# philips/janus

Hardware: AMD Instinct MI355X
Metric: reports prepared+aggregated/sec (helper, Prio3Histogram len=256) at 1/2/4/8 GPUs (higher is better)
Workload: dtype u32 limbs (Field128 mod-p integer arithmetic); 1 GPU; Prio3Histogram length=256 chunk_length=16 helper prepare_init+prepare_shares_to_prepare_message+prepare_next+aggregate, 1 segment; reports_per_gpu=1048576, global_batch=1048576, parallelism=dp1 (report shards; RCCL all-gather + mod-p combine)

## Files before the change

janus_amd/csrc/prio3_prepare.hip:

```cpp
#include <hip/hip_runtime.h>

#include <algorithm>

#include "prio3_host.h"
#include "prio3_query_sum.h"

#ifndef XOFD_BLOCK
#define XOFD_BLOCK 256
#endif
#ifndef XOFD_OCC
#define XOFD_OCC 3
#endif
template <class F>
__device__ __forceinline__ void xof_body(const DevParams& p, const InPtrs& in, const Scratch& sc,
                                         const uint32_t r) {
  if (r >= p.n) return;
  constexpr uint32_t ES = F::ES;
  uint32_t flag = p.force_slow;
  uint32_t nonce[4], km[4], kp[4], kb[4] = {0, 0, 0, 0};
  load16(in.nonces + 16 * (size_t)r, nonce);
  const uint8_t* hs = in.helper + (size_t)r * p.helper_share_len;
  load16(hs, km);
  load16(hs + 16, kp);
  const bool JR = p.jr_len > 0;
// ... 1051 lines not shown
  }
  return any != 0;
}

template <class F>
__device__ __forceinline__ void query_body(const DevParams& p, const InPtrs& in, const Scratch& sc,
                                           const OutPtrs& out, const uint32_t r) {
  typedef typename F::T T;
  if (r >= p.n) return;
  if (p.redo) {
    if (sc.flag[r] != 2) return;
  } else if (p.slow_defer && sc.flag[r]) {
    return;
  }
  const size_t ld = p.ld;
  const uint32_t A = p.arity;
  uint8_t status = PRIO3_STATUS_FINISHED;
  const T t = ldf<F>(sc.qr, 0, ld, r);
  T v, pt;
  if (!flp_query_lane<F>(p, sc.meas, sc.proofs, sc.jr, t, sc.Lbuf, sc.PVbuf, sc.acc, r, v, pt))
    status = PRIO3_STATUS_PREP_INIT;
  const uint8_t* lps = in.leader + (size_t)r * p.prep_share_len;
  bool decode_ok = true;
  auto lv = [&](uint32_t e) {
    T x = F::load(lps, e);
    if (!F::lt_p(x)) decode_ok = false;
    return x;
  };
  const T V0 = F::add(lv(0), v);
  T G = F::zero();
  if (p.kind == PRIO3_COUNT) {
    T a = F::add(lv(1), F::load(sc.acc, 0 * ld + r));
    T b = F::add(lv(2), F::load(sc.acc, 1 * ld + r));
    G = F::mul(a, b);
  } else if (p.kind == PRIO3_SUM) {
    T a = F::add(lv(1), F::load(sc.acc, r));
    G = F::sub(F::mul(a, a), a);
  } else {
    for (uint32_t j = 0; j < p.chunk; j++) {
      T a = F::add(lv(1 + 2 * j), F::load(sc.acc, (size_t)(2 * j) * ld + r));
      T b = F::add(lv(2 + 2 * j), F::load(sc.acc, (size_t)(2 * j + 1) * ld + r));
      G = F::add(G, F::mul(a, b));
    }
  }
  const T PT = F::add(lv(A + 1), pt);
  if (status == PRIO3_STATUS_FINISHED) {
    if (!decode_ok)
      status = PRIO3_STATUS_PREP_SHARE_DECODE;
    else if (!F::is_zero(V0) || !F::eq(G, PT))
      status = PRIO3_STATUS_PREP_MSG;
  }
  uint32_t msg[4] = {0, 0, 0, 0};
  if (p.jr_len > 0) {
    uint32_t lpart[4], hpart[4];
    load16(lps + (size_t)p.verifier_len * F::ES, lpart);
    uint4 hp = sc.part[r];
    hpart[0] = hp.x;
    hpart[1] = hp.y;
    hpart[2] = hp.z;
    hpart[3] = hp.w;
    KState s;
    kzero(s);
    Msg m;
    msg_zero(m);
    msg_dst(m, p.dst[6]);
    msg_bytes16(m, 25, lpart);
    msg_bytes16(m, 41, hpart);
    msg_absorb_final(s, m, 57);
    uint4 cor = sc.corrected[r];
    msg[0] = kword(s, 0);
    msg[1] = kword(s, 1);
    msg[2] = kword(s, 2);
    msg[3] = kword(s, 3);
    if (status == PRIO3_STATUS_FINISHED &&
        (msg[0] != cor.x || msg[1] != cor.y || msg[2] != cor.z || msg[3] != cor.w))
      status = PRIO3_STATUS_PREP_NEXT;
    if (status != PRIO3_STATUS_FINISHED) msg[0] = msg[1] = msg[2] = msg[3] = 0;
    ((uint4*)out.prep_msgs)[r] = make_uint4(msg[0], msg[1], msg[2], msg[3]);
  }
  out.status[r] = status;
  if (p.kind == PRIO3_SUM) {
    T acc = F::zero(), pw = F::one();
    for (uint32_t i = 0; i < p.meas_len; i++) {
      acc = F::add(acc, F::mul(pw, ldf<F>(sc.meas, i, ld, r)));
      pw = F::add(pw, pw);
    }
    F::store(sc.out, r, acc);
  } else if (p.kind == PRIO3_SUMVEC) {
    for (uint32_t e = 0; e < p.out_len; e++) {
      T acc = F::zero(), pw = F::one();
      for (uint32_t b = 0; b < p.bits; b++) {
        acc = F::add(acc, F::mul(pw, ldf<F>(sc.meas, e * p.bits + b, ld, r)));
        pw = F::add(pw, pw);
      }
      F::store(sc.out, (size_t)e * ld + r, acc);
    }
  }
}
template <class F>
__global__ __launch_bounds__(256) void k_query(DevParams p, InPtrs in, Scratch sc, OutPtrs out) {
  query_body<F>(p, in, sc, out, blockIdx.x * blockDim.x + threadIdx.x);
}

template <class F>
__global__ __launch_bounds__(256) void k_prep_gen(DevParams p, InPtrs in, Scratch sc, OutPtrs out) {
  const uint32_t r = blockIdx.x * blockDim.x + threadIdx.x;
  xof_body<F>(p, in, sc, r);
  query_body<F>(p, in, sc, out, r);
}

template <class F>
__global__ __launch_bounds__(64) void k_slow_redo_gen(DevParams p, InPtrs in, Scratch sc,
                                                      OutPtrs out) {
  const uint32_t r0 = (blockIdx.x * blockDim.x + threadIdx.x) * REDO_RPL;
  if (r0 >= p.n || !redo_any(p, sc, r0)) return;
  const uint8_t* fl = sc.flag + r0;
  for (uint32_t i = 0; i < REDO_RPL && r0 + i < p.n; i++)
    if (fl[i]) {
      xof_slow_one<F>(p, in, sc, r0 + i);
      query_body<F>(p, in, sc, out, r0 + i);
    }
}

template <int GS>
__global__ __launch_bounds__(256) void k_query_ps(DevParams p, InPtrs in, Scratch sc,
                                                  OutPtrs out) {
  typedef Fp128 F;
  typedef f128 T;
  const uint32_t r = blockIdx.x * blockDim.x + threadIdx.x;
  if (r >= p.n) return;
  const size_t ld = p.ld;
  const uint32_t P = p.P, A = p.arity, C = p.chunk, M = p.meas_len, K = p.calls;
  uint8_t status = PRIO3_STATUS_FINISHED;
  const T t = ldf<F>(sc.qr, 0, ld, r);
  {
    T tp = t;
    for (uint32_t l = 0; l < p.logP; l++) tp = F::mul(tp, tp);
    if (F::eq(tp, F::one())) status = PRIO3_STATUS_PREP_INIT;
  }
  {
    T pw = FC<F>::invP(p);
    for (uint32_t e = 0; e < P; e++) {
      F::store(sc.Lbuf, (size_t)bitrev(e, p.logP) * ld + r, pw);
      pw = F::mul(pw, t);
    }
    dft_lane<F>(p, sc.Lbuf, r, P, p.logP);
    for (uint32_t e = 0; e < P; e++) {
      T q = ldf<F>(sc.proofs, A + e, ld, r);
      if (e + P < p.glen) q = F::add(q, ldf<F>(sc.proofs, A + e + P, ld, r));
      F::store(sc.PVbuf, (size_t)bitrev(e, p.logP) * ld + r, q);
    }
    dft_lane<F>(p, sc.PVbuf, r, P, p.logP);
  }
  auto Lc = [&](uint32_t c) { return ldf<F>(sc.Lbuf, (P - c) & (P - 1), ld, r); };
  T pt = F::zero();
  for (uint32_t e = p.glen; e-- > 0;) pt = F::add(F::mul(pt, t), ldf<F>(sc.proofs, A + e, ld, r));
  const T r0 = ldf<F>(sc.jr, 0, ld, r);
  T rC = F::one();
  for (uint32_t j = 0; j < C; j++) rC = F::mul(rC, r0);
  T sumL = F::zero(), range = F::zero();
  {
    T rk = F::one();
    for (uint32_t k = 0; k < K; k++) {
      const T L = Lc(k + 1);
      sumL = F::add(sumL, L);
      range = F::add(range, ldf<F>(sc.PVbuf, k + 1, ld, r));
      F::store(sc.beta, (size_t)k * ld + r, F::mul(L, rk));
      rk = F::mul(rk, rC);
    }
  }
  const T L0 = Lc(0);
  const T half = FC<F>::half(p);
  const T halfL = F::mul(half, sumL);
  const uint8_t* lps = in.leader + (size_t)r * p.prep_share_len;
  bool decode_ok = true;
  auto lv = [&](uint32_t e) {
    T x = F::load(lps, e);
    if (!F::lt_p(x)) decode_ok = false;
    return x;
  };
  T S = F::zero(), G = F::zero(), rj = r0;
  const T Z = F::zero();
  for (uint32_t jg = 0; jg < C; jg += GS) {
    T Aa[GS], Bb[GS];
#pragma unroll
    for (int q = 0; q < GS; q++) Aa[q] = Bb[q] = Z;
    auto ldm = [&](uint32_t k, int q) {
      const uint32_t i = k * C + jg + (uint32_t)q;
      return ldf<F>(sc.meas, (jg + q < C && i < M) ? i : 0, ld, r);
    };
    T be_n = ldf<F>(sc.beta, 0, ld, r), L_n = Lc(1), mn[GS];
#pragma unroll
    for (int q = 0; q < GS; q++) mn[q] = ldm(0, q);
#pragma unroll 1
    for (uint32_t k = 0; k < K; k++) {
      const T be = be_n, L = L_n;
      T mc[GS];
#pragma unroll
      for (int q = 0; q < GS; q++) mc[q] = mn[q];
      const uint32_t kn = k + 1 < K ? k + 1 : k;
      be_n = ldf<F>(sc.beta, kn, ld, r);
      L_n = Lc(kn + 1);
#pragma unroll
      for (int q = 0; q < GS; q++) mn[q] = ldm(kn, q);
      const uint32_t base = k * C + jg;
#pragma unroll
      for (int q = 0; q < GS; q++) {
        const bool valid = (jg + q < C) && (base + q < M);
        const T m = F::sel(valid, mc[q], Z);
        Aa[q] = F::add(Aa[q], F::mul(be, m));
        Bb[q] = F::add(Bb[q], F::mul(L, m));
        S = F::add(S, m);
      }
    }
#pragma unroll
    for (int q = 0; q < GS; q++) {
      const uint32_t j = jg + q;
      const bool valid = j < C;
      const uint32_t jj = valid ? j : 0;
      const T f0 = F::add(F::mul(ldf<F>(sc.proofs, 2 * jj, ld, r), L0), F::mul(rj, Aa[q]));
      const T f1 = F::sub(F::add(F::mul(ldf<F>(sc.proofs, 2 * jj + 1, ld, r), L0), Bb[q]), halfL);
      const T prod = F::mul(F::add(lv(1 + 2 * jj), f0), F::add(lv(2 + 2 * jj), f1));
      G = F::add(G, F::sel(valid, prod, Z));
      rj = F::sel(valid, F::mul(rj, r0), rj);
    }
  }
  T v;
  if (p.kind == PRIO3_SUMVEC) {
    v = range;
  } else {
    const T r1 = ldf<F>(sc.jr, 1, ld, r);
    v = F::add(F::mul(r1, range), F::mul(F::mul(r1, r1), F::sub(S, half)));
  }
  const T V0 = F::add(lv(0), v);
  const T PT = F::add(lv(A + 1), pt);
  if (status == PRIO3_STATUS_FINISHED) {
    if (!decode_ok)
      status = PRIO3_STATUS_PREP_SHARE_DECODE;
    else if (!F::is_zero(V0) || !F::eq(G, PT))
      status = PRIO3_STATUS_PREP_MSG;
  }
  uint32_t lpart[4], hpart[4];
  load16(lps + (size_t)p.verifier_len * F::ES, lpart);
  {
    uint4 hp = sc.part[r];
    hpart[0] = hp.x;
    hpart[1] = hp.y;
    hpart[2] = hp.z;
    hpart[3] = hp.w;
  }
  KState s;
  kzero(s);
  Msg mm;
  msg_zero(mm);
  msg_dst(mm, p.dst[6]);
  msg_bytes16(mm, 25, lpart);
  msg_bytes16(mm, 41, hpart);
  msg_absorb_final(s, mm, 57);
  uint4 cor = sc.corrected[r];
  uint32_t msg[4] = {kword(s, 0), kword(s, 1), kword(s, 2), kword(s, 3)};
  if (status == PRIO3_STATUS_FINISHED &&
      (msg[0] != cor.x || msg[1] != cor.y || msg[2] != cor.z || msg[3] != cor.w))
    status = PRIO3_STATUS_PREP_NEXT;
  if (status != PRIO3_STATUS_FINISHED) msg[0] = msg[1] = msg[2] = msg[3] = 0;
  ((uint4*)out.prep_msgs)[r] = make_uint4(msg[0], msg[1], msg[2], msg[3]);
  out.status[r] = status;
  if (p.kind == PRIO3_SUMVEC) {
    for (uint32_t e = 0; e < p.out_len; e++) {
      T acc = F::zero(), pw = F::one();
      for (uint32_t b = 0; b < p.bits; b++) {
        acc = F::add(acc, F::mul(pw, ldf<F>(sc.meas, e * p.bits + b, ld, r)));
        pw = F::add(pw, pw);
      }
      F::store(sc.out, (size_t)e * ld + r, acc);
    }
  }
}

template <int GS, int PP, int LEADER = 0>
__device__ __forceinline__ void query_h_body(const DevParams& p, const InPtrs& in, const Scratch& sc,
                                             const OutPtrs& out, const uint32_t r) {
  typedef Fp128 F;
  typedef f128 T;
  constexpr int LOGP = PP <= 2 ? 1 : PP <= 4 ? 2 : PP <= 8 ? 3 : PP <= 16 ? 4 : 5;
  if (r >= p.n) return;
  if constexpr (!LEADER) {
    if (p.redo) {
      if (sc.flag[r] != 2) return;
    } else if (p.slow_defer && sc.flag[r]) {
      return;
    }
  } else {
    if (p.redo) {
      if (!sc.flag[r]) return;
    } else if (p.slow_defer && sc.flag[r]) {
      return;
    }
  }
  const size_t ld = p.ld;
  const uint32_t A = p.arity, C = p.chunk, M = p.meas_len, K = p.calls;
  uint8_t status = LEADER ? out.status[r] : PRIO3_STATUS_FINISHED;
  uint8_t* lout = LEADER ? out.prep_msgs + (size_t)r * p.prep_share_len : nullptr;
  const T t = ldf<F>(sc.qr, 0, ld, r);
  T L0, sumL = F::zero();
  auto store_L = [&](int idx, const T& val) {
    const uint32_t c = (uint32_t)((PP - idx) & (PP - 1));
    if (c == 0) {
      L0 = val;
    } else if (c <= K) {
      F::store(sc.Lbuf, (size_t)c * ld + r, val);
      sumL = F::add(sumL, val);
    }
  };
  if constexpr (PP <= 16) {
    T x[PP];
    T pw = FC<F>::invP(p);
#pragma unroll
    for (int e = 0; e < PP; e++) {
      x[__builtin_bitreverse32(e) >> (32 - LOGP)] = pw;
      pw = F::mul(pw, t);
    }
    if (F::eq(pw, FC<F>::invP(p))) status = PRIO3_STATUS_PREP_INIT;
    dft_reg<PP, LOGP>(p, x, 1);
#pragma unroll
    for (int k = 0; k < PP; k++) store_L(k, x[k]);
  } else {
    static_assert(PP == 32, "PP must be <= 32");
    T t8 = t;
#pragma unroll
    for (int i = 0; i < 3; i++) t8 = F::mul(t8, t8);
    const T t16 = F::mul(t8, t8);
    const T t32 = F::mul(t16, t16);
    if (F::eq(t32, F::one())) status = PRIO3_STATUS_PREP_INIT;
    const T ip = FC<F>::invP(p);
    const T a = F::add(F::one(), t16), b = F::sub(F::one(), t16);
    const T c = F::mul(t8, a), wd = F::mul(F::mul(t8, b), F::from_words(p.tw128[8]));
#pragma unroll
    for (int ph = 0; ph < 4; ph++) {
      const T g = ph == 0 ? F::add(a, c) : ph == 1 ? F::add(b, wd) : ph == 2 ? F::sub(a, c)
                                                                              : F::sub(b, wd);
      T x[8];
      T pw = F::mul(ip, g);
      const T ratio = ph == 0 ? t : F::mul(t, F::from_words(p.tw128[ph]));
#pragma unroll
      for (int e = 0; e < 8; e++) {
        x[__builtin_bitreverse32(e) >> 29] = pw;
        if (e + 1 < 8) pw = F::mul(pw, ratio);
      }
      dft_reg<8, 3>(p, x, 4);
#pragma unroll
      for (int k = 0; k < 8; k++) store_L(4 * k + ph, x[k]);
    }
  }
  T pt = F::zero(), range;
  {
    constexpr int GLEN = 2 * (PP - 1) + 1, NB = (GLEN + 7) / 8;
    T pw[8];
    pw[0] = F::one();
    pw[1] = t;
#pragma unroll
    for (int i = 2; i < 8; i++) pw[i] = F::mul(pw[i - 1], t);
    const T t8b = F::mul(pw[7], t);
    mac128 R;
    mac_zero(R);
    auto ldc = [&](int e) { return ldf<F>(sc.proofs, A + (e < GLEN ? e : 0), ld, r); };
    T cb[8];
#pragma unroll
    for (int i = 0; i < 8; i++) cb[i] = ldc(8 * (NB - 1) + i);
#pragma unroll 1
    for (int q = NB - 1; q >= 0; q--) {
      T cn[8];
      const int qn = q > 0 ? q - 1 : 0;
#pragma unroll
      for (int i = 0; i < 8; i++) cn[i] = ldc(8 * qn + i);
      mac128 S;
      mac_zero(S);
#pragma unroll
      for (int i = 0; i < 8; i++) {
        const int e = 8 * q + i;
        if (e < GLEN) {
          mac_add(S, cb[i], pw[i]);
          mac_add(R, cb[i], F::from_words(p.sigma128[e & (PP - 1)]));
        }
        cb[i] = cn[i];
      }
      const T sq = mac_reduce_f(S);
      pt = q == NB - 1 ? sq : F::add(F::mul(pt, t8b), sq);
    }
    range = mac_reduce_f(R);
  }
  const T r0 = ldf<F>(sc.jr, 0, ld, r);
  {
    T rC = F::one(), sq = r0;
    for (uint32_t e = C; e; e >>= 1) {
      if (e & 1) rC = F::mul(rC, sq);
      if (e > 1) sq = F::mul(sq, sq);
    }
    T rk = F::one();
    for (uint32_t k0 = 0; k0 < K; k0 += 8) {
      T lb[8];
#pragma unroll
      for (int q = 0; q < 8; q++) lb[q] = ldf<F>(sc.Lbuf, k0 + q < K ? k0 + q + 1 : 1, ld, r);
#pragma unroll
      for (int q = 0; q < 8; q++) {
        if (k0 + q < K) {
          F::store(sc.beta, (size_t)(k0 + q) * ld + r, F::mul(lb[q], rk));
          rk = F::mul(rk, rC);
        }
      }
    }
  }
  const T half = FC<F>::half(p);
  const T halfL = F::mul(half, sumL);
  const uint8_t* lps = in.leader + (size_t)r * p.prep_share_len;
  bool decode_ok = true;
  auto lv = [&](uint32_t e) {
    T x = F::load(lps, e);
    if (!F::lt_p(x)) decode_ok = false;
    return x;
  };
  sum128 Ssum;
  sum_zero(Ssum);
  T G = F::zero(), rj = r0;
  for (uint32_t jg = 0; jg < C; jg += GS) {
    mac128 Aa[GS], Bb[GS];
    T mc[GS];
#pragma unroll
    for (int q = 0; q < GS; q++) {
      mac_zero(Aa[q]);
      mac_zero(Bb[q]);
    }
    auto fetch = [&](uint32_t k, T* dst) {
#pragma unroll
      for (int q = 0; q < GS; q++) {
        const uint32_t i = k * C + jg + q;
        const bool valid = (k < K) && (jg + q < C) && (i < M);
        const uint32_t msk = valid ? 0xffffffffu : 0u;
        const uint4 v = ((const uint4*)sc.meas)[(size_t)(valid ? i : 0) * ld + r];
        dst[q] = mk128(v.x & msk, v.y & msk, v.z & msk, v.w & msk);
      }
    };
    fetch(0, mc);
    T be = ldf<F>(sc.beta, 0, ld, r), Lk = ldf<F>(sc.Lbuf, 1, ld, r);
#pragma unroll 1
    for (uint32_t k = 0; k < K; k++) {
      T mn[GS];
      fetch(k + 1, mn);
      const uint32_t kn = k + 1 < K ? k + 1 : k;
      const T be_n = ldf<F>(sc.beta, kn, ld, r), L_n = ldf<F>(sc.Lbuf, kn + 1, ld, r);
#pragma unroll
      for (int q = 0; q < GS; q++) {
        mac_add(Aa[q], be, mc[q]);
        mac_add(Bb[q], Lk, mc[q]);
        sum_add(Ssum, mc[q]);
      }
#pragma unroll
      for (int q = 0; q < GS; q++) mc[q] = mn[q];
      be = be_n;
      Lk = L_n;
    }
    mac128 Gq;
    mac_zero(Gq);
#pragma unroll
    for (int q = 0; q < GS; q++) {
      const uint32_t j = jg + q;
      if (j < C) {
        mac_add(Bb[q], ldf<F>(sc.proofs, 2 * j + 1, ld, r), L0);
        const T f1 = F::sub(mac_reduce_f(Bb[q]), halfL);
        const T Aq = mac_reduce_f(Aa[q]);
        mac128 F0;
        mac_zero(F0);
        mac_add(F0, ldf<F>(sc.proofs, 2 * j, ld, r), L0);
        mac_add(F0, rj, Aq);
        const T f0 = mac_reduce_f(F0);
        if constexpr (LEADER) {
          F::store(lout, 1 + 2 * j, f0);
          F::store(lout, 2 + 2 * j, f1);
        } else {
          mac_add(Gq, F::add(lv(1 + 2 * j), f0), F::add(lv(2 + 2 * j), f1));
        }
        rj = F::mul(rj, r0);
      }
    }
    if constexpr (!LEADER) G = F::add(G, mac_reduce_f(Gq));
  }
  const T S = sum_reduce(Ssum);
  T v;
  if (p.kind == PRIO3_SUMVEC) {
    v = range;
  } else {
    const T r1 = ldf<F>(sc.jr, 1, ld, r);
    v = F::add(F::mul(r1, range), F::mul(F::mul(r1, r1), F::sub(S, half)));
  }
  if constexpr (LEADER) {
    F::store(lout, 0, v);
    F::store(lout, A + 1, pt);
    *(uint4*)(lout + (size_t)p.verifier_len * F::ES) = sc.part[r];
    out.status[r] = status;
  } else {
  const T V0 = F::add(lv(0), v);
  const T PT = F::add(lv(A + 1), pt);
  if (status == PRIO3_STATUS_FINISHED) {
    if (!decode_ok)
      status = PRIO3_STATUS_PREP_SHARE_DECODE;
    else if (!F::is_zero(V0) || !F::eq(G, PT))
      status = PRIO3_STATUS_PREP_MSG;
  }
  uint32_t lpart[4], msg[4];
  load16(lps + (size_t)p.verifier_len * F::ES, lpart);
  if (!prep_msg_check(p, in, sc, r, lpart, msg) && status == PRIO3_STATUS_FINISHED)
    status = PRIO3_STATUS_PREP_NEXT;
  if (status != PRIO3_STATUS_FINISHED) msg[0] = msg[1] = msg[2] = msg[3] = 0;
  ((uint4*)out.prep_msgs)[r] = make_uint4(msg[0], msg[1], msg[2], msg[3]);
  out.status[r] = status;
  }
  if (p.kind == PRIO3_SUMVEC) {
    for (uint32_t e = 0; e < p.out_len; e++) {
      T acc = F::zero(), pw = F::one();
      for (uint32_t b = 0; b < p.bits; b++) {
        acc = F::add(acc, F::mul(pw, ldf<F>(sc.meas, e * p.bits + b, ld, r)));
        pw = F::add(pw, pw);
      }
      F::store(sc.out, (size_t)e * ld + r, acc);
    }
  }
}
template <int GS, int PP, int LEADER = 0>
__global__ __launch_bounds__(256, 3) void k_query_h(DevParams p, InPtrs in, Scratch sc,
                                                  OutPtrs out) {
  query_h_body<GS, PP, LEADER>(p, in, sc, out, blockIdx.x * blockDim.x + threadIdx.x);
}

template <bool FUSE, bool PULL = false>
__global__ __launch_bounds__(XOFD_BLOCK, 3) void k_prep_h(DevParams p, InPtrs in, Scratch sc,
                                                   OutPtrs out) {
  const uint32_t r = blockIdx.x * blockDim.x + threadIdx.x;
  xofd_body<FUSE, false, PULL>(p, in, sc, r);
  query_h_body<2, 32>(p, in, sc, out, r);
}

template <int PP>
__global__ __launch_bounds__(256, 3) void k_leader_prep(DevParams p, InPtrs in, Scratch sc,
                                                        OutPtrs out, uint32_t* wpart,
                                                        uint32_t* wseg) {
  const uint32_t r = blockIdx.x * blockDim.x + threadIdx.x;
  leader_jr_body(p, in, sc, out.status, wpart, wseg, r);
  query_h_body<2, PP, 1>(p, in, sc, out, r);
}

template <int NPH>
__global__ __launch_bounds__(256, 3) void k_prep_sum(DevParams p, InPtrs in, Scratch sc,
                                                     OutPtrs out) {
  const uint32_t r = blockIdx.x * blockDim.x + threadIdx.x;
  xofd_body<false, false>(p, in, sc, r);
  qsum::query_sum_body<NPH, 0>(p, in, sc, out, r);
}

template <int PP>
__global__ __launch_bounds__(64) void k_slow_redo(DevParams p, InPtrs in, Scratch sc, OutPtrs out) {
  const uint32_t r0 = (blockIdx.x * blockDim.x + threadIdx.x) * REDO_RPL;
  if (r0 >= p.n || !redo_any(p, sc, r0)) return;
  const uint8_t* fl = sc.flag + r0;
  for (uint32_t i = 0; i < REDO_RPL && r0 + i < p.n; i++)
    if (fl[i]) {
      xof_slow_one<Fp128>(p, in, sc, r0 + i);
      query_h_body<2, PP>(p, in, sc, out, r0 + i);
    }
}

template <int NPH>
__global__ __launch_bounds__(64) void k_slow_redo_sum(DevParams p, InPtrs in, Scratch sc,
                                                      OutPtrs out) {
  const uint32_t r0 = (blockIdx.x * blockDim.x + threadIdx.x) * REDO_RPL;
  if (r0 >= p.n || !redo_any(p, sc, r0)) return;
  const uint8_t* fl = sc.flag + r0;
  for (uint32_t i = 0; i < REDO_RPL && r0 + i < p.n; i++)
    if (fl[i]) {
      xof_slow_one<Fp128>(p, in, sc, r0 + i);
      qsum::query_sum_body<NPH, 0>(p, in, sc, out, r0 + i);
    }
}


static void fp_sub_sizes(const prio3_engine* e, uint32_t n, uint32_t cap, bool wide,
                         uint32_t& nsub, uint32_t& sub) {
  nsub = (n + cap - 1) / cap;
  sub = std::min(cap, (((n + nsub - 1) / nsub) + 255) & ~255u);
  if (wide && e->fp_round && nsub > 1) {
    const uint32_t Q = (uint32_t)e->n_cu * 4u * 2u * 8u;
    const uint32_t s2 = sub / Q * Q;
    if (s2 > 0 && n - (nsub - 1) * s2 <= cap) sub = s2;
  }
}

template <class F>
static void launch_xof_slow(const prio3_engine* e, const DevParams& p, const InPtrs& in,
                            const Scratch& sc, hipStream_t st) {
  (void)e;
  k_xof_slow<F><<<slow_blocks(p.n), 64, 0, st>>>(p, in, sc);
}

bool fusable(const prio3_engine* e) {
  return e->fuse_acc && e->dp.kind == PRIO3_HISTOGRAM && e->dp.jr_len &&
         (42 + e->dp.meas_len * 16) / 168 >= 2;
}

static int ensure_side_streams(prio3_engine* e) {
  while (e->side.size() < 2) {
    hipStream_t s2;
    hipEvent_t j;
    HIPCHK(hipStreamCreateWithFlags(&s2, hipStreamNonBlocking));
    HIPCHK(hipEventCreateWithFlags(&j, hipEventDisableTiming));
    e->side.push_back(s2);
    e->side_ev.push_back(j);
  }
  if (!e->fork_ev) HIPCHK(hipEventCreateWithFlags(&e->fork_ev, hipEventDisableTiming));
  return PRIO3_OK;
}

static bool prep_fused_takes(const prio3_engine* e, const DevParams& dp, bool fuse) {
  if (e->force_generic) return false;
  const bool ps = dp.kind == PRIO3_HISTOGRAM || dp.kind == PRIO3_SUMVEC;
  const bool dual = dp.es == 16 && dp.jr_len && (42 + dp.meas_len * 16) / 168 >= 2;
  if (dp.kind == PRIO3_SUM) return dual && !fuse && query_sum_takes(dp);
  return ps && dual && dp.P == 32;
}

enum : int { DEFER_NONE = 0, DEFER_QH = 1, DEFER_SUM = 2, DEFER_GEN64 = 3 };
static int launch_prepare(prio3_engine* e, const DevParams& base, uint32_t c0, uint32_t n,
                          InPtrs in, OutPtrs out, Scratch sc, hipStream_t st, bool fuse,
                          int* deferred, bool pair = false) {
  DevParams dp = base;
  dp.n = n;
  dp.force_slow = (uint32_t)e->force_slow;
  dp.slow_defer = 0;
  dp.redo = 0;
  const size_t es = dp.es;
  in.nonces += 16 * (size_t)c0;
  if (in.pub) in.pub += (size_t)dp.public_share_len * c0;
  in.helper += (size_t)dp.helper_share_len * c0;
  in.leader += (size_t)dp.prep_share_len * c0;
  if (in.vk_slot) in.vk_slot += c0;
  out.prep_msgs += (size_t)(dp.kind == PRIO3_SUMVEC_F64_MP ? 32 : 16) * c0;
  out.status += c0;
  void** soa[] = {&sc.meas, &sc.proofs, &sc.jr, &sc.qr, &sc.Lbuf, &sc.PVbuf, &sc.acc, &sc.out,
                  &sc.beta};
  for (auto q : soa)
    if (*q) *q = (uint8_t*)*q + es * c0;
  sc.part += c0;
  sc.corrected += c0;
  sc.flag += c0;
  if (sc.seg) sc.seg += c0;
  if (sc.wseg) sc.wseg += c0 / 64;
  if (sc.wpart) sc.wpart += (size_t)(c0 / 64) * dp.meas_len * 8;
  const uint32_t blocks = (n + 255) / 256;
  const uint32_t xblocks = (n + XOFD_BLOCK - 1) / XOFD_BLOCK;
  if (dp.kind == PRIO3_SUMVEC_F64_MP) {
    int rc = PRIO3_OK;
    TIMED(e, st, "k_mp64_prepare", (rc = launch_mp64(e, n, dp.ld, in, out, sc, st)));
    return rc;
  }
  if (dp.kind == PRIO3_FPVEC_BOUNDED_L2) {
    uint32_t nsub, sub;
    const bool qwide = !e->force_generic && fpvec_query_wide_takes(dp);
    fp_sub_sizes(e, n, dp.ld, qwide, nsub, sub);
    for (uint32_t si = 0; si < nsub; si++) {
      const uint32_t s0 = si * sub;
      DevParams q = dp;
      q.n = si + 1 < nsub ? sub : n - s0;
      InPtrs qi = in;
      qi.nonces += 16 * (size_t)s0;
      qi.pub += (size_t)dp.public_share_len * s0;
      qi.helper += (size_t)dp.helper_share_len * s0;
      qi.leader += (size_t)dp.prep_share_len * s0;
      if (qi.vk_slot) qi.vk_slot += s0;
      OutPtrs qo = out;
      qo.prep_msgs += 16 * (size_t)s0;
      qo.status += s0;
      Scratch qs = sc;
      qs.out = (uint8_t*)sc.out + es * s0;
      const uint32_t qb = (q.n + 255) / 256;
      const bool dual = (42 + dp.meas_len * 16) / 168 >= 2;
      q.trunc_xof = dual ? 1u : 0u;
      bool paired = false;
      if (dual) TIMED(e, st, "k_xof_pair", (paired = launch_xof_pair(q, qi, qs, st)));
      if (!paired && dual)
        TIMED(e, st, "k_xofd",
              (k_xofd<false, true><<<(q.n + XOFD_BLOCK - 1) / XOFD_BLOCK, XOFD_BLOCK, 0, st>>>(
                  q, qi, qs)));
      else if (!paired)
        TIMED(e, st, "k_xof", (k_xof<Fp128><<<qb, 256, 0, st>>>(q, qi, qs)));
      TIMED(e, st, "k_xof_slow", launch_xof_slow<Fp128>(e, q, qi, qs, st));
      if (qwide)
        TIMED(e, st, "k_query_fpw", launch_fpvec_query(q, qi, qs, qo, st, true, false));
      else
        TIMED(e, st, "k_query_fp", launch_fpvec_query(q, qi, qs, qo, st, false, false));
    }
    return PRIO3_OK;
  }
  if (dp.es == 16) {
    const bool ps = dp.kind == PRIO3_HISTOGRAM || dp.kind == PRIO3_SUMVEC;
    const bool wide = ps && !e->force_generic && dp.P != 32 && query_wide_takes(dp);
    const bool dual = dp.jr_len && (42 + dp.meas_len * 16) / 168 >= 2;
    dp.trunc_xof = dp.kind == PRIO3_SUMVEC && wide && dual && !fuse ? 1u : 0u;
    if (prep_fused_takes(e, dp, fuse)) {
      dp.slow_defer = 1u;
      if (dp.kind == PRIO3_SUM) {
        if (deferred) *deferred = DEFER_SUM;
        switch (dp.P) {
          case 16: TIMED(e, st, "k_prep_sum", (k_prep_sum<1><<<blocks, 256, 0, st>>>(dp, in, sc, out))); break;
          case 32: TIMED(e, st, "k_prep_sum", (k_prep_sum<2><<<blocks, 256, 0, st>>>(dp, in, sc, out))); break;
          case 64: TIMED(e, st, "k_prep_sum", (k_prep_sum<4><<<blocks, 256, 0, st>>>(dp, in, sc, out))); break;
          default: TIMED(e, st, "k_prep_sum", (k_prep_sum<8><<<blocks, 256, 0, st>>>(dp, in, sc, out))); break;
        }
      } else {
        if (deferred) *deferred = DEFER_QH;
        const bool pl = in.leader_src != nullptr;
        bool paired = false;
        if (pair)
          TIMED(e, st, "k_prep_hp", (paired = launch_prep_pair(dp, in, sc, out, st, fuse, pl)));
        if (paired) {
        } else if (fuse && pl)
          TIMED(e, st, "k_prep_h", (k_prep_h<true, true><<<xblocks, XOFD_BLOCK, 0, st>>>(dp, in, sc, out)));
        else if (fuse)
          TIMED(e, st, "k_prep_h", (k_prep_h<true><<<xblocks, XOFD_BLOCK, 0, st>>>(dp, in, sc, out)));
        else if (pl)
          TIMED(e, st, "k_prep_h", (k_prep_h<false, true><<<xblocks, XOFD_BLOCK, 0, st>>>(dp, in, sc, out)));
        else
          TIMED(e, st, "k_prep_h", (k_prep_h<false><<<xblocks, XOFD_BLOCK, 0, st>>>(dp, in, sc, out)));
      }
      return PRIO3_OK;
    }
    if (dual) {
      if (fuse)
        TIMED(e, st, "k_xofd", (k_xofd<true><<<xblocks, XOFD_BLOCK, 0, st>>>(dp, in, sc)));
      else if (dp.trunc_xof)
        TIMED(e, st, "k_xofd", (k_xofd<false, true><<<xblocks, XOFD_BLOCK, 0, st>>>(dp, in, sc)));
      else
        TIMED(e, st, "k_xofd", (k_xofd<false><<<xblocks, XOFD_BLOCK, 0, st>>>(dp, in, sc)));
    } else {
      TIMED(e, st, "k_xof_a", (k_xof_a<Fp128><<<blocks, 256, 0, st>>>(dp, in, sc)));
      TIMED(e, st, "k_jrpart", (k_jrpart<false><<<blocks, 256, 0, st>>>(dp, in, sc)));
    }
    const bool qh_path =
        ps && !e->force_generic && !wide && (dp.P == 32 || dp.P == 16 || dp.P == 8);
    dp.slow_defer = qh_path ? 1u : 0u;
    if (qh_path && deferred) *deferred = DEFER_QH;
    if (!qh_path) TIMED(e, st, "k_xof_slow", launch_xof_slow<Fp128>(e, dp, in, sc, st));
    bool done = false;
    if (wide) TIMED(e, st, "k_query_w", (done = launch_query_wide(dp, in, sc, out, st)));
    if (done) {
    } else if (qh_path && dp.P == 32)
      TIMED(e, st, "k_query_h", (k_query_h<2, 32><<<blocks, 256, 0, st>>>(dp, in, sc, out)));
    else if (qh_path && dp.P == 16)
      TIMED(e, st, "k_query_h", (k_query_h<2, 16><<<blocks, 256, 0, st>>>(dp, in, sc, out)));
    else if (qh_path && dp.P == 8)
      TIMED(e, st, "k_query_h", (k_query_h<2, 8><<<blocks, 256, 0, st>>>(dp, in, sc, out)));
    else if (ps)
      TIMED(e, st, "k_query_ps", (k_query_ps<4><<<blocks, 256, 0, st>>>(dp, in, sc, out)));
    else {
      bool qs = false;
      if (!e->force_generic && query_sum_takes(dp))
        TIMED(e, st, "k_query_sum", (qs = launch_query_sum(dp, in, sc, out, st)));
      if (!qs) TIMED(e, st, "k_query", (k_query<Fp128><<<blocks, 256, 0, st>>>(dp, in, sc, out)));
    }
  } else {
    dp.slow_defer = 1u;
    if (deferred) *deferred = DEFER_GEN64;
    TIMED(e, st, "k_prep_gen", (k_prep_gen<Fp64><<<blocks, 256, 0, st>>>(dp, in, sc, out)));
  }
  return PRIO3_OK;
}

static int launch_slow_redo(prio3_engine* e, const DevParams& base, uint32_t n, InPtrs in,
                            OutPtrs out, Scratch sc, hipStream_t st, int family) {
  DevParams dp = base;
  dp.n = n;
  dp.force_slow = (uint32_t)e->force_slow;
  dp.trunc_xof = 0;
  dp.slow_defer = 1;
  dp.redo = 1;
  const uint32_t g = redo_blocks(n);
  if (family == DEFER_GEN64) {
    TIMED(e, st, "k_slow_redo", (k_slow_redo_gen<Fp64><<<g, 64, 0, st>>>(dp, in, sc, out)));
  } else if (family == DEFER_SUM) {
    switch (dp.P) {
      case 16: TIMED(e, st, "k_slow_redo", (k_slow_redo_sum<1><<<g, 64, 0, st>>>(dp, in, sc, out))); break;
      case 32: TIMED(e, st, "k_slow_redo", (k_slow_redo_sum<2><<<g, 64, 0, st>>>(dp, in, sc, out))); break;
      case 64: TIMED(e, st, "k_slow_redo", (k_slow_redo_sum<4><<<g, 64, 0, st>>>(dp, in, sc, out))); break;
// ... 196 lines not shown
```

Before: 177.9 million reports/s.

## Spill live values to scratch and pipeline measurement loads with scalar offsets

Values that stay live across the long inner loop (L0, halfL, pt, range) now go to scratch buffers and are reloaded afterward, which lowers register pressure. Row loads use a per-lane base address plus a wave-uniform offset taken with readfirstlane, so address arithmetic can live in scalar registers. The inner loop is rewritten as a software pipeline with a remainder prologue and an unrolled steady state. The finalization loads for proofs, leader shares and jr are issued early so their latency is hidden. The cost is extra global memory traffic and reliance on compiler barriers and offsets being wave-uniform.

```diff
diff --git a/janus_amd/csrc/prio3_prepare.hip b/janus_amd/csrc/prio3_prepare.hip
--- a/janus_amd/csrc/prio3_prepare.hip
+++ b/janus_amd/csrc/prio3_prepare.hip
@@ -1377,11 +1377,11 @@
   uint8_t status = LEADER ? out.status[r] : PRIO3_STATUS_FINISHED;
   uint8_t* lout = LEADER ? out.prep_msgs + (size_t)r * p.prep_share_len : nullptr;
   const T t = ldf<F>(sc.qr, 0, ld, r);
-  T L0, sumL = F::zero();
+  T sumL = F::zero();
   auto store_L = [&](int idx, const T& val) {
     const uint32_t c = (uint32_t)((PP - idx) & (PP - 1));
     if (c == 0) {
-      L0 = val;
+      F::store(sc.Lbuf, r, val);
     } else if (c <= K) {
       F::store(sc.Lbuf, (size_t)c * ld + r, val);
       sumL = F::add(sumL, val);
@@ -1464,6 +1464,8 @@
     }
     range = mac_reduce_f(R);
   }
+  F::store(sc.PVbuf, (size_t)1 * ld + r, pt);
+  F::store(sc.PVbuf, (size_t)2 * ld + r, range);
   const T r0 = ldf<F>(sc.jr, 0, ld, r);
   {
     T rC = F::one(), sq = r0;
@@ -1486,7 +1488,7 @@
     }
   }
   const T half = FC<F>::half(p);
-  const T halfL = F::mul(half, sumL);
+  F::store(sc.PVbuf, r, F::mul(half, sumL));
   const uint8_t* lps = in.leader + (size_t)r * p.prep_share_len;
   bool decode_ok = true;
   auto lv = [&](uint32_t e) {
@@ -1497,69 +1499,133 @@
   sum128 Ssum;
   sum_zero(Ssum);
   T G = F::zero(), rj = r0;
+  uint64_t lane = (uint64_t)sc.meas + (uint64_t)r * F::ES;
+  asm("" : "+v"(lane));
   for (uint32_t jg = 0; jg < C; jg += GS) {
     mac128 Aa[GS], Bb[GS];
-    T mc[GS];
 #pragma unroll
     for (int q = 0; q < GS; q++) {
       mac_zero(Aa[q]);
       mac_zero(Bb[q]);
     }
-    auto fetch = [&](uint32_t k, T* dst) {
+    constexpr int WIRE_AHEAD = 1;
+    struct wire_ops {
+      T m[GS];
+      T be, L;
+    };
+    auto ldrow = [&](const void* base, uint32_t e) {
+      const uint64_t off = ((uint64_t)base - (uint64_t)sc.meas) + (uint64_t)e * ld * F::ES;
+      const uint64_t offu =
+          ((uint64_t)(uint32_t)__builtin_amdgcn_readfirstlane((int)(uint32_t)(off >> 32)) << 32) |
+          (uint32_t)__builtin_amdgcn_readfirstlane((int)(uint32_t)off);
+      typedef uint32_t u32x4 __attribute__((ext_vector_type(4)));
+      const u32x4 v = *(const __attribute__((address_space(1))) u32x4*)(lane + offu);
+      return mk128(v.x, v.y, v.z, v.w);
+    };
+    const uint32_t Klast = K ? K - 1 : 0;
+    auto issue = [&](uint32_t k, wire_ops& s) {
 #pragma unroll
       for (int q = 0; q < GS; q++) {
         const uint32_t i = k * C + jg + q;
         const bool valid = (k < K) && (jg + q < C) && (i < M);
+        s.m[q] = ldrow(sc.meas, i & (valid ? 0xffffffffu : 0u));
+      }
+      const uint32_t kc = min(k, Klast);
+      s.be = ldrow(sc.beta, kc);
+      s.L = ldrow(sc.Lbuf, kc + 1);
+    };
+    auto use = [&](uint32_t k, wire_ops& s) {
+#pragma unroll
+      for (int q = 0; q < GS; q++)
+        asm volatile(""
+                     : "+v"(s.m[q].w[0]), "+v"(s.m[q].w[1]), "+v"(s.m[q].w[2]), "+v"(s.m[q].w[3])
+                     :
+                     : "memory");
+#pragma unroll
+      for (int q = 0; q < GS; q++) {
+        const bool valid = (jg + q < C) && (k * C + jg + q < M);
         const uint32_t msk = valid ? 0xffffffffu : 0u;
-        const uint4 v = ((const uint4*)sc.meas)[(size_t)(valid ? i : 0) * ld + r];
-        dst[q] = mk128(v.x & msk, v.y & msk, v.z & msk, v.w & msk);
+        const T mc = mk128(s.m[q].w[0] & msk, s.m[q].w[1] & msk, s.m[q].w[2] & msk,
+                           s.m[q].w[3] & msk);
+        mac_add(Aa[q], s.be, mc);
+        mac_add(Bb[q], s.L, mc);
+        sum_add(Ssum, mc);
       }
     };
-    fetch(0, mc);
-    T be = ldf<F>(sc.beta, 0, ld, r), Lk = ldf<F>(sc.Lbuf, 1, ld, r);
+    constexpr int NS = WIRE_AHEAD + 1;
+    wire_ops ws[NS];
+    uint32_t k = __builtin_amdgcn_readfirstlane(0);
+    asm volatile("" : "+s"(k));
+#pragma unroll
+    for (int u = 0; u < WIRE_AHEAD; u++) issue(k + u, ws[u]);
 #pragma unroll 1
-    for (uint32_t k = 0; k < K; k++) {
-      T mn[GS];
-      fetch(k + 1, mn);
-      const uint32_t kn = k + 1 < K ? k + 1 : k;
-      const T be_n = ldf<F>(sc.beta, kn, ld, r), L_n = ldf<F>(sc.Lbuf, kn + 1, ld, r);
-#pragma unroll
-      for (int q = 0; q < GS; q++) {
-        mac_add(Aa[q], be, mc[q]);
-        mac_add(Bb[q], Lk, mc[q]);
-        sum_add(Ssum, mc[q]);
-      }
-#pragma unroll
-      for (int q = 0; q < GS; q++) mc[q] = mn[q];
-      be = be_n;
-      Lk = L_n;
-    }
+    for (uint32_t e = K % NS; e; e--, k++) {
+      issue(k + WIRE_AHEAD, ws[WIRE_AHEAD]);
+      use(k, ws[0]);
+#pragma unroll
+      for (int u = 0; u < WIRE_AHEAD; u++) ws[u] = ws[u + 1];
+    }
+#pragma unroll 1
+    for (; k < K; k += NS) {
+#pragma unroll
+      for (int u = 0; u < NS; u++) {
+        issue(k + u + WIRE_AHEAD, ws[(u + WIRE_AHEAD) % NS]);
+        use(k + u, ws[u]);
+      }
+    }
+    T sd[2 * GS], lw[2 * GS], r0f;
+    auto fin_load = [&](int q) {
+      const uint32_t jc = jg + q < C ? jg + q : jg;
+      if constexpr (!LEADER) {
+        lw[2 * q] = F::load(lps, 1 + 2 * jc);
+        lw[2 * q + 1] = F::load(lps, 2 + 2 * jc);
+      }
+    };
+    const T L0 = ldrow(sc.Lbuf, 0), halfL = ldrow(sc.PVbuf, 0);
+#pragma unroll
+    for (int q = 0; q < GS; q++) {
+      const uint32_t jc = jg + q < C ? jg + q : jg;
+      sd[2 * q + 1] = ldrow(sc.proofs, 2 * jc + 1);
+      sd[2 * q] = ldrow(sc.proofs, 2 * jc);
+    }
+    fin_load(0);
+    asm volatile("" ::: "memory");
     mac128 Gq;
     mac_zero(Gq);
 #pragma unroll
     for (int q = 0; q < GS; q++) {
       const uint32_t j = jg + q;
-      if (j < C) {
-        mac_add(Bb[q], ldf<F>(sc.proofs, 2 * j + 1, ld, r), L0);
-        const T f1 = F::sub(mac_reduce_f(Bb[q]), halfL);
+      if (q == 0 || j < C) {
+        mac_add(Bb[q], sd[2 * q + 1], L0);
+        T f1 = F::sub(mac_reduce_f(Bb[q]), halfL);
+        if (q == 0) {
+          asm volatile("" : "+v"(f1.w[0])::"memory");
+          r0f = ldrow(sc.jr, 0);
+#pragma unroll
+          for (int q2 = 1; q2 < GS; q2++) fin_load(q2);
+          asm volatile("" ::: "memory");
+        }
         const T Aq = mac_reduce_f(Aa[q]);
         mac128 F0;
         mac_zero(F0);
-        mac_add(F0, ldf<F>(sc.proofs, 2 * j, ld, r), L0);
+        mac_add(F0, sd[2 * q], L0);
         mac_add(F0, rj, Aq);
         const T f0 = mac_reduce_f(F0);
         if constexpr (LEADER) {
           F::store(lout, 1 + 2 * j, f0);
           F::store(lout, 2 + 2 * j, f1);
         } else {
-          mac_add(Gq, F::add(lv(1 + 2 * j), f0), F::add(lv(2 + 2 * j), f1));
+          if (!F::lt_p(lw[2 * q]) || !F::lt_p(lw[2 * q + 1])) decode_ok = false;
+          mac_add(Gq, F::add(lw[2 * q], f0), F::add(lw[2 * q + 1], f1));
         }
-        rj = F::mul(rj, r0);
+        rj = F::mul(rj, r0f);
       }
     }
     if constexpr (!LEADER) G = F::add(G, mac_reduce_f(Gq));
   }
   const T S = sum_reduce(Ssum);
+  pt = ldf<F>(sc.PVbuf, 1, ld, r);
+  range = ldf<F>(sc.PVbuf, 2, ld, r);
   T v;
   if (p.kind == PRIO3_SUMVEC) {
     v = range;
```

Result: faster. 179.8 million reports/s, median of 6 (+1.0%).
